# TritonDataCenter/node-zkstream

Measured on AMD Instinct MI355X. Metric: ZK ops/sec (whole node) + p50 get() RTT, 1M-znode synthetic tree, higher is better.
Workload: dtype uint8

## Files before the change

csrc/kernels/tree.hip:

```cpp
#include "zk_tree.h"
#include "zk_frame_rows.h"

namespace zk {

__global__ __launch_bounds__(TR_T) void tree_fill_k(ZkTree t, int64_t n0,
                                                   int64_t n,
                                                   const int32_t* __restrict__ nkids,
                                                   int64_t now_ms) {
  const int64_t v = n0 + (int64_t)blockIdx.x * TR_T + threadIdx.x;
  if (v >= n) return;
  const ZkNodeStore& s = t.store;
  uint8_t* slot = s.slab + s.slot_off[v];
  const int32_t dl = s.data_len[v];
  fill_stat(slot, v + 1, v + 1, now_ms, now_ms, 0, nkids[v], 0, 0, dl,
            nkids[v], v + 1);
  st_be32(slot + 68, 0);
  st_be32(slot + ZK_SLOT_LEN, dl > 0 ? dl : -1);
  t.cn[v] = cn_pack(nkids[v], nkids[v]);
  t.pzxid[v] = v + 1;
  t.eph[v] = 0;
  t.dirty[v] = 0;
}

__global__ __launch_bounds__(TR_T) void free_count_k(ZkTree t,
                                                    int64_t* __restrict__ bsum) {
  __shared__ int32_t c[TR_T / 64];
  const int64_t nn = min(t.counters[TC_NODES], t.store.cap);
  const int64_t v = (int64_t)blockIdx.x * TR_T + threadIdx.x;
  const bool f = v < nn && t.node_parent[v] == NODE_FREE;
  const uint64_t m = __ballot(f);
  if ((threadIdx.x & 63) == 0) c[threadIdx.x >> 6] = __popcll(m);
  __syncthreads();
  if (threadIdx.x == 0) {
    int64_t s = 0;
    for (int k = 0; k < TR_T / 64; ++k) s += c[k];
    bsum[blockIdx.x] = s;
  }
}

__global__ __launch_bounds__(TR_T) void free_scatter_k(
    ZkTree t, const int64_t* __restrict__ bbase,
    const int64_t* __restrict__ total) {
  __shared__ int32_t c[TR_T / 64];
  const int64_t head = t.counters[TC_FREE_HEAD];
  const int64_t nn = min(t.counters[TC_NODES], t.store.cap);
  const int64_t v = (int64_t)blockIdx.x * TR_T + threadIdx.x;
  const bool f = v < nn && t.node_parent[v] == NODE_FREE;
  const uint64_t m = __ballot(f);
  const int w = threadIdx.x >> 6;
  if ((threadIdx.x & 63) == 0) c[w] = __popcll(m);
  __syncthreads();
  int64_t r = bbase[blockIdx.x] +
              __builtin_amdgcn_mbcnt_hi((uint32_t)(m >> 32),
                                        __builtin_amdgcn_mbcnt_lo((uint32_t)m, 0));
  for (int k = 0; k < w; ++k) r += c[k];
  if (f) t.free_list[(head + r) % t.free_cap] = v;
  if (blockIdx.x == 0 && threadIdx.x == 0) {
    t.counters[TC_FREE_TAIL] = head + *total;
    t.counters[TC_FREE_PUB] = head + *total;
  }
}

__global__ __launch_bounds__(TR_T) void tree_build_k(ZkTree t, int64_t n0,
                                                    int64_t n) {
  const int64_t v = n0 + (int64_t)blockIdx.x * TR_T + threadIdx.x;
  if (v >= n || t.node_parent[v] == NODE_FREE) return;
  tree_insert(t, v, t.path_arena + t.node_path_off[v], t.node_path_len[v],
              t.store.data_len[v]);
}

}

extern "C" {

int zk_tree_fill(const ZkTree* t, int64_t n0, int64_t n, const int32_t* nkids,
                 int64_t now_ms, hipStream_t st) {
  if (n <= n0) return 0;
  const int64_t m = n - n0;
  zk::tree_fill_k<<<(unsigned)((m + zk::TR_T - 1) / zk::TR_T), zk::TR_T, 0,
                    st>>>(*t, n0, n, nkids, now_ms);
  ZK_LAUNCH_CHECK();
  return 0;
}

int64_t zk_tree_free_workspace(int64_t cap) {
  const int64_t nb = (cap + zk::TR_T - 1) / zk::TR_T;
  return 2 * nb + 8 + zk_scan_workspace(nb);
}

int zk_tree_free_compact(const ZkTree* t, int64_t* ws, hipStream_t st) {
  const int64_t nb = (t->store.cap + zk::TR_T - 1) / zk::TR_T;
  if (nb <= 0) return 0;
  int64_t* bsum = ws;
  int64_t* bbase = ws + nb;
  int64_t* total = ws + 2 * nb;
  zk::free_count_k<<<(unsigned)nb, zk::TR_T, 0, st>>>(*t, bsum);
  ZK_LAUNCH_CHECK();
  int rc = zk_scan_excl_i64(bsum, bbase, nb, total, ws + 2 * nb + 8, st);
  if (rc) return rc;
  zk::free_scatter_k<<<(unsigned)nb, zk::TR_T, 0, st>>>(*t, bbase, total);
  ZK_LAUNCH_CHECK();
  return 0;
}

int zk_tree_ht_reset(const ZkTree* t, hipStream_t st) {
  return hipMemsetAsync(t->ht, 0, (size_t)(t->mask + 1) * zk::HT_W * 8, st);
}

int zk_tree_build(const ZkTree* t, int64_t n0, int64_t n, hipStream_t st) {
  if (n <= n0) return 0;
  const int64_t m = n - n0;
  zk::tree_build_k<<<(unsigned)((m + zk::TR_T - 1) / zk::TR_T), zk::TR_T, 0,
                     st>>>(*t, n0, n);
  ZK_LAUNCH_CHECK();
  return 0;
}

}

namespace zk {

ZK_DEV void put_seq10(uint8_t* d, int32_t x) {
  uint32_t u = (uint32_t)x;
#pragma unroll
  for (int k = 9; k >= 0; --k) { d[k] = (uint8_t)('0' + u % 10); u /= 10; }
}

struct Lane {
  int32_t op, err, pl, dl, flags, dlen;
  int64_t node, zx, par, slot;
  const uint8_t* path;
};

ZK_DEV int64_t served_reply_size(int32_t op, int32_t err, int32_t dl,
                                 int32_t rpl) {
  const int64_t sz = 4 + 16;
  if (err != ERR_OK) return sz;
  switch (op) {
    case OP_GET_DATA: return sz + 4 + max(dl, 0) + STAT_BYTES;
    case OP_EXISTS: case OP_SET_DATA: return sz + STAT_BYTES;
    case OP_CREATE: return sz + 4 + max(rpl, 0);
    default: return sz;
  }
}

ZK_DEV int32_t seq_num(const ZkTree& t, int64_t i) {
  if (t.seqno == nullptr) return -1;
  const int64_t x = t.seqno[i];
  return x < 0 ? -1 : (int32_t)(uint32_t)x;
}
ZK_DEV int64_t seq_par(const ZkTree& t, int64_t i) {
  return t.seqno == nullptr || t.seqno[i] < 0 ? -1 : t.seqno[i] >> 32;
}

ZK_DEV int32_t do_create(const ZkTree& t, Lane& L, const uint8_t* data,
                         int32_t nacl, int64_t session, int64_t now_ms,
                         int64_t v, int64_t i) {
  const ZkNodeStore& s = t.store;
  const bool eph = L.flags & CF_EPHEMERAL, seq = L.flags & CF_SEQUENTIAL;
  const int32_t pre = seq ? seq_num(t, i) : -1;
  if (nacl <= 0) return ERR_INVALID_ACL;
  if (v < 0) return ERR_SYSTEM;
  const int64_t vpo = t.node_path_off[v];
  const int64_t vso = s.slot_off[v];
  const uint8_t* path = L.path;
  const int32_t pl = L.pl;
  int32_t cut = pl - 1;
  while (cut > 0 && path[cut] != '/') --cut;
  const int64_t par = cut > 0 ? tree_find(t, path, cut) : -1;
  if (cut > 0 && par < 0) return ERR_NO_NODE;
  if (par >= 0 && t.eph[par] != 0)
    return ERR_NO_CHILDREN_FOR_EPHEMERALS;
  const int32_t npl = pl + (seq ? 10 : 0);
  const bool taken = seq && par >= 0 && pre < 0;
  const int32_t seqno = !seq || par < 0 ? 0
                        : pre >= 0      ? pre
                                        : cn_cver(cn_add(t, par, 1, 1));
  uint8_t* pd = t.path_arena + vpo;
  copy_bytes(pd, path, pl);
  if (seq) put_seq10(pd + pl, seqno);
  const int32_t dl = L.dl;
  uint8_t* slot = s.slab + vso;
  fill_stat(slot, L.zx, L.zx, now_ms, now_ms, 0, 0, 0, eph ? session : 0, dl,
            0, L.zx);
  st_be32(slot + ZK_SLOT_LEN, dl > 0 ? dl : -1);
  copy_bytes(slot + ZK_SLOT_DATA, data, dl);
  t.node_path_len[v] = npl;
  s.data_len[v] = dl;
  t.cn[v] = 0;
  t.pzxid[v] = L.zx;
  t.node_parent[v] = par;
  t.node_pw[v] = pw_pack(pd - t.path_arena, npl);
  const int64_t ins = pre >= 0 ? tree_insert<true>(t, v, pd, npl, dl, vso)
                               : tree_insert(t, v, pd, npl, dl, vso);
  if (ins != v) {
    if (taken) cn_add(t, par, 0, -1);
    return ins < 0 ? ERR_SYSTEM : ERR_NODE_EXISTS;
  }
  t.eph[v] = eph ? session : 0;
  if (par >= 0) {
    if (seq) {
      atomicMax((unsigned long long*)&t.pzxid[par], (unsigned long long)L.zx);
    } else {
      parent_touch(t, par, 1, true, L.zx);
    }
  }
  L.par = par;
  L.node = v;
  L.slot = s.slot_off[v];
  return ERR_OK;
}

struct ServeSegs : ZkSegs {};
static_assert(TR_T == FR_T, "a workgroup per block of FR_T frames");
template <bool PARSE, bool RO, bool TILES, bool MS = false, bool DEFER = false>
ZK_DEV void tree_serve_body(
    const ZkTree& t, const uint8_t* __restrict__ rx, const ZkReqOut& q,
    const int64_t* __restrict__ foff, const int32_t* __restrict__ flen,
    const int64_t* __restrict__ n_dev, int64_t ncap, int32_t* __restrict__ r_op,
    int32_t* __restrict__ r_xid, int32_t* __restrict__ r_err,
    int64_t* __restrict__ r_node, int64_t* __restrict__ r_zxid,
    int64_t* __restrict__ r_path_off, int32_t* __restrict__ r_path_len,
    int64_t* __restrict__ r_slot, int64_t* __restrict__ r_sizes,
    int64_t* __restrict__ r_bsum, int64_t session, int64_t now_ms,
    const uint8_t* __restrict__ rank, int32_t pass, int32_t last_pass,
    int64_t snap_base, int64_t snap_cap, int64_t* __restrict__ snap_top,
    int32_t wslot, int64_t* __restrict__ fired, const ZkFrameTiles* T,
    int64_t* __restrict__ rows_off, int32_t* __restrict__ rows_len,
    const ServeSegs* M = nullptr) {
  session = sess_of(t, session);
  const uint32_t blk = xcd_remap(blockIdx.x, gridDim.x);
  const int64_t i = (int64_t)blk * TR_T + threadIdx.x;
  const bool in_batch = i < ncap && i < *n_dev;
  int64_t fo = 0;
  int32_t fl = 0;
  if (TILES) {
    __shared__ FrLds rows;
    const int64_t nf = *n_dev;
    if (fr_row(*T, blk, nf < ncap ? nf : ncap, rows, fo, fl)) {
      rows_off[i] = fo;
      rows_len[i] = fl;
    }
    fr_housekeep(*T);
  }
  const int32_t rb = rank != nullptr && in_batch ? (int32_t)rank[i] : 0;
  const int32_t rk = rb & ORD_RANK;
  const bool live = in_batch && (rk == pass || (last_pass && rk > pass));
  int32_t ms_err = ERR_OK;
  if (MS && live) {
    const int64_t sg = M->f_seg[i];
    if (*M->bad != 0 || sg < 0 || sg >= M->S) {
      ms_err = ERR_SYSTEM;
    } else {
      session = sess_of(t, M->sessions[sg]);
      wslot = M->wslots[sg];
      if (M->seg_state[sg] == 1) ms_err = ERR_SESSION_EXPIRED;
    }
  }
  const bool refused = live && (rk > pass || (MS && ms_err != ERR_OK));
  ReqFields rq{ST_BAD_DECODE, 0, OP_PING, 0, 0, 0, 0, -1, -1, -1, 0};
  if (live) {
    if (PARSE) {
      rq = TILES ? parse_request(rx, fo, fl)
                 : parse_request(rx, foff[i], flen[i]);
    } else {
      rq.status = q.status[i];
      rq.xid = q.xid[i];
      rq.op = q.opcode[i];
      rq.arg = q.arg[i];
      rq.pl = q.path_len[i];
      rq.dl = q.data_len[i];
      rq.vc = q.vec_count[i];
      rq.poff = q.path_off[i];
      rq.doff = q.data_off[i];
    }
  }
  const bool ok_req = live && !refused && rq.status == ST_OK;
  const ZkNodeStore& s = t.store;
  Lane L;
  L.op = live ? rq.op : OP_PING;
  L.err = refused ? (MS && ms_err != ERR_OK ? ms_err : ERR_SYSTEM)
                  : (live && !ok_req ? ERR_BAD_ARGUMENTS : ERR_OK);
  L.node = -1;
  L.slot = -1;
  L.dlen = 0;
  L.par = -1;
  L.flags = 0;
  L.path = nullptr;
  L.pl = L.dl = 0;
  if (ok_req) {
    L.path = rx + rq.poff;
    L.pl = rq.pl;
    L.dl = max(rq.dl, 0);
    L.flags = rq.arg;
  }
  const bool write = ok_req && (L.op == OP_CREATE || L.op == OP_SET_DATA ||
                                L.op == OP_DELETE);
  const int64_t zbase = t.counters[TC_ZXID];
  L.zx = write ? zbase + i + 1 : zbase;
  const bool create = !RO && ok_req && L.op == OP_CREATE;
  int64_t v = -1;
  int32_t npl = 0, cap = 0;
  if (create) {
    npl = L.pl + ((L.flags & CF_SEQUENTIAL) ? 10 : 0);
    cap = max(L.dl, 128);
  }
  if (RO && ok_req && L.op != OP_GET_DATA && L.op != OP_EXISTS)
    L.err = ERR_UNIMPLEMENTED;
  if (!RO) {
    const int64_t pub = t.counters[TC_FREE_PUB];
    const int64_t h = block_ticket(&t.counters[TC_FREE_HEAD], create);
    if (create && h < pub) v = t.free_list[h % t.free_cap];
    const bool fresh = create && v < 0;
    const int64_t nv = block_ticket(&t.counters[TC_NODES], fresh);
    if (fresh && nv < s.cap) v = nv;
    const bool new_path = v >= 0 && (fresh || npl > t.node_path_cap[v]);
    const bool new_slot = v >= 0 && (fresh || cap > s.slot_cap[v]);
    const int32_t pcap = (npl + 15) & ~15;
    const int64_t po = wave_bytes(&t.counters[TC_PATH_TOP],
                                  new_path ? pcap : 0);
    const int64_t sb = new_slot ? slot_bytes(cap) : 0;
    const int64_t so = wave_bytes(&t.counters[TC_SLAB_TOP], sb);
    if (new_path) {
      if (po + pcap <= t.path_cap) {
        t.node_path_off[v] = po;
        t.node_path_len[v] = npl;
        t.node_path_cap[v] = pcap;
      } else {
        t.node_path_len[v] = 0;
        t.node_path_cap[v] = 0;
      }
    }
    if (new_slot) {
      if (so + sb <= t.slab_cap) {
        s.slot_off[v] = so;
        s.slot_cap[v] = cap;
      } else {
        s.slot_cap[v] = -1;
      }
    }
    if (v >= 0 && ((new_path && po + pcap > t.path_cap) ||
                   (new_slot && so + sb > t.slab_cap))) {
      L.err = ERR_SYSTEM;
    }
  }
  int64_t freed = -1;
  bool numbered = !RO && live && seq_num(t, i) >= 0;
  if (ok_req && L.err == ERR_OK) {
    switch (L.op) {
      case OP_GET_DATA: case OP_EXISTS:
        {
          const Found f = tree_lookup<true>(t, L.path, L.pl);
          L.node = f.node;
          L.slot = f.slot;
          L.dlen = f.dlen;
        }
        if (L.node < 0) L.err = ERR_NO_NODE;
        break;
      case OP_SET_DATA: {
        const Found f = tree_lookup(t, L.path, L.pl);
        const int64_t node = f.node;
        if (node < 0) { L.err = ERR_NO_NODE; break; }
        L.slot = f.slot;
        if (L.dl > s.slot_cap[node]) { L.err = ERR_BAD_ARGUMENTS; break; }
        uint8_t* slot = s.slab + L.slot;
        unsigned int* ver = (unsigned int*)(slot + 32);
        const int32_t want = L.flags;
        unsigned int old = *ver, cmp;
        do {
          cmp = old;
          if (want != -1 && cmp != bswap32((uint32_t)want)) break;
          old = atomicCAS(ver, cmp, bswap32(bswap32(cmp) + 1));
        } while (old != cmp);
        if (old != cmp || (want != -1 && cmp != bswap32((uint32_t)want))) {
          L.err = ERR_BAD_VERSION;
          break;
        }
        copy_bytes(slot + ZK_SLOT_DATA, rx + rq.doff, L.dl);
        st_be32(slot + ZK_SLOT_LEN, L.dl > 0 ? L.dl : -1);
        s.data_len[node] = L.dl;
        ent_set_dlen(t, f.ent, L.dl);
        st_be64(slot + 8, L.zx);
        st_be64(slot + 24, now_ms);
        st_be32(slot + 52, L.dl);
        L.node = node;
        break;
      }
      case OP_CREATE:
        L.err = do_create(t, L, rx + rq.doff, rq.vc, session,
                          now_ms, v, i);
        if (L.err == ERR_OK) numbered = false;
        if (L.err == ERR_OK && r_path_off != nullptr) {
          r_path_off[i] = t.node_path_off[v];
          r_path_len[i] = t.node_path_len[v];
        }
        break;
      case OP_DELETE: {
        const Found f = tree_lookup(t, L.path, L.pl);
        const int64_t node = f.node, so = f.slot;
        if (node < 0) { L.err = ERR_NO_NODE; break; }
        const int32_t nkids = cn_nchild(__hip_atomic_load(
            &t.cn[node], __ATOMIC_RELAXED, __HIP_MEMORY_SCOPE_AGENT));
        const int32_t want = L.flags;
        if (want != -1 && ld_be32(s.slab + so + 32) != want) {
          L.err = ERR_BAD_VERSION;
          break;
        }
        if (nkids > 0) {
          L.err = ERR_NOT_EMPTY;
          break;
        }
        if (!tree_erase_at(t, f.ent, node)) { L.err = ERR_NO_NODE; break; }
        L.par = t.node_parent[node];
        if (L.par >= 0) parent_touch(t, L.par, -1, true, L.zx);
        t.eph[node] = 0;
        freed = node;
        break;
      }
      case OP_SYNC: case OP_PING:
        break;
      case OP_SET_WATCHES:
        break;
      default:
        L.err = ERR_UNIMPLEMENTED;
    }
  }
  if (numbered)
    cn_add(t, seq_par(t, i),
           MS && ms_err == ERR_SYSTEM && !(DEFER && rk == ORD_RANK) ? -1 : 0,
           -1);
  if (t.wt_key != nullptr && ok_req) {
    const bool wflag = rq.arg == 1;
    if (L.op == OP_GET_DATA && wflag && L.err == ERR_OK) {
      wt_arm(t, L.path, L.pl, WK_DATA, wslot);
    } else if (L.op == OP_EXISTS && wflag &&
               (L.err == ERR_OK || L.err == ERR_NO_NODE)) {
      wt_arm(t, L.path, L.pl, WK_DATA, wslot);
    } else if (L.err == ERR_OK && (L.op == OP_SET_DATA ||
                                   L.op == OP_CREATE ||
                                   L.op == OP_DELETE)) {
      const int64_t node = L.op == OP_DELETE ? freed : L.node;
      const int64_t pw = t.node_pw[node];
      const int64_t ppw = L.par >= 0 ? t.node_pw[L.par] : 0;
      const uint8_t* np = node_path(t, pw);
      const int32_t nl = pw_len(pw);
      uint64_t m0 = wt_fire(t, np, nl, WK_DATA), m1 = 0, m2 = 0;
      if (L.op == OP_DELETE) m1 = wt_fire(t, np, nl, WK_CHILD) & ~m0;
      if (L.op != OP_SET_DATA && L.par >= 0)
        m2 = wt_fire(t, node_path(t, ppw), pw_len(ppw), WK_CHILD);
      if (fired != nullptr) {
        int64_t* f = fired + (int64_t)WT_REC * i;
        f[0] = (int64_t)m0;
        f[1] = (int64_t)m1;
        f[2] = (int64_t)m2;
        f[3] = pw;
        f[4] = ppw;
      }
    }
  }
  if (rank != nullptr) {
    const bool snap = (rb & ORD_SNAP) && live && L.err == ERR_OK &&
                      (L.op == OP_GET_DATA || L.op == OP_EXISTS ||
                       L.op == OP_SET_DATA);
    const int64_t dl = snap && L.op == OP_GET_DATA ? L.dlen : 0;
    const int64_t sb = snap ? slot_bytes((int32_t)dl) : 0;
    const int64_t so = wave_bytes(snap_top, sb);
    if (snap) {
      if (so + sb <= snap_cap) {
        copy_bytes(s.slab + snap_base + so, s.slab + L.slot,
                   (int32_t)(ZK_SLOT_DATA + dl));
        L.slot = snap_base + so;
      } else {
        L.err = ERR_SYSTEM;
      }
    }
  }
  if (create && L.err != ERR_OK && v >= 0) freed = v;
  if (!RO) {
    wave_free(t, freed);
    wave_mark_dirty(t, L.err == ERR_OK ? L.par
                       : DEFER && numbered ? seq_par(t, i) : -1);
  }
  if (r_sizes != nullptr) {
    __shared__ int64_t sm[TR_T / 64 + 1];
    int64_t sz = 0;
    if (live) {
      const bool get = L.err == ERR_OK && L.op == OP_GET_DATA;
      const bool mk = L.err == ERR_OK && L.op == OP_CREATE;
      sz = served_reply_size(L.op, L.err, get ? L.dlen : 0,
                             mk ? t.node_path_len[L.node] : 0);
      r_sizes[i] = sz;
    } else if (in_batch && rk < pass) {
      sz = r_sizes[i];
    } else if (!in_batch && i < ncap) {
      r_sizes[i] = 0;
    }
    int64_t tot;
    block_excl_scan(sz, sm, &tot);
    if (threadIdx.x == 0) r_bsum[blk] = tot;
  }
  if (!live) return;
  r_op[i] = L.op;
  r_xid[i] = rq.xid;
  r_err[i] = L.err;
  r_node[i] = L.op == OP_DELETE ? -1 : L.node;
  r_zxid[i] = L.zx;
  if (r_slot != nullptr) r_slot[i] = L.op == OP_DELETE ? -1 : L.slot;
}

template <bool PARSE, bool RO = false>
__global__ __launch_bounds__(TR_T) void tree_serve_k(
    ZkTree t, const uint8_t* __restrict__ rx, ZkReqOut q,
    const int64_t* __restrict__ foff, const int32_t* __restrict__ flen,
    const int64_t* __restrict__ n_dev, int64_t ncap, int32_t* __restrict__ r_op,
    int32_t* __restrict__ r_xid, int32_t* __restrict__ r_err,
    int64_t* __restrict__ r_node, int64_t* __restrict__ r_zxid,
    int64_t* __restrict__ r_path_off, int32_t* __restrict__ r_path_len,
    int64_t* __restrict__ r_slot, int64_t* __restrict__ r_sizes,
    int64_t* __restrict__ r_bsum, int64_t session, int64_t now_ms,
    const uint8_t* __restrict__ rank, int32_t pass, int32_t last_pass,
    int64_t snap_base, int64_t snap_cap, int64_t* __restrict__ snap_top,
    int32_t wslot, int64_t* __restrict__ fired) {
  tree_serve_body<PARSE, RO, false>(
      t, rx, q, foff, flen, n_dev, ncap, r_op, r_xid, r_err, r_node, r_zxid,
      r_path_off, r_path_len, r_slot, r_sizes, r_bsum, session, now_ms, rank,
      pass, last_pass, snap_base, snap_cap, snap_top, wslot, fired, nullptr,
      nullptr, nullptr);
}

template <bool RO>
__global__ __launch_bounds__(TR_T) void tree_serve_tiles_k(
    ZkTree t, ZkFrameTiles T, int64_t* __restrict__ rows_off,
    int32_t* __restrict__ rows_len, const int64_t* __restrict__ n_dev,
    int64_t ncap, ZkServeOut o, int64_t session, int64_t now_ms,
    int32_t wslot, int64_t* __restrict__ fired) {
  tree_serve_body<true, RO, true>(
      t, T.buf, ZkReqOut{}, nullptr, nullptr, n_dev, ncap, o.opcode, o.xid,
      o.err, o.node, o.zxid, o.path_off, o.path_len, o.slot, o.sizes,
      o.block_sums, session, now_ms, nullptr, 0, 1, 0, 0, nullptr, wslot,
      fired, &T, rows_off, rows_len);
}

template <bool PARSE>
__global__ __launch_bounds__(TR_T) void tree_serve_sess_k(
    ZkTree t, const uint8_t* __restrict__ rx, ZkReqOut q,
    const int64_t* __restrict__ foff, const int32_t* __restrict__ flen,
    const int64_t* __restrict__ n_dev, int64_t ncap, ZkServeOut o,
    int64_t now_ms, const uint8_t* __restrict__ rank, int32_t pass,
    int32_t last_pass, int64_t snap_base, int64_t snap_cap,
    int64_t* __restrict__ snap_top, int64_t* __restrict__ fired,
    ServeSegs M) {
  tree_serve_body<PARSE, false, false, true>(
      t, rx, q, foff, flen, n_dev, ncap, o.opcode, o.xid, o.err, o.node,
      o.zxid, o.path_off, o.path_len, o.slot, o.sizes, o.block_sums, 0,
      now_ms, rank, pass, last_pass, snap_base, snap_cap, snap_top, -1, fired,
      nullptr, nullptr, nullptr, &M);
}

__global__ __launch_bounds__(TR_T) void tree_serve_sess_defer_k(
    ZkTree t, const uint8_t* __restrict__ rx, ZkReqOut q,
    const int64_t* __restrict__ n_dev, int64_t ncap, ZkServeOut o,
    int64_t now_ms, const uint8_t* __restrict__ rank, int32_t pass,
    int32_t last_pass, int64_t snap_base, int64_t snap_cap,
    int64_t* __restrict__ snap_top, int64_t* __restrict__ fired,
    ServeSegs M) {
  tree_serve_body<false, false, false, true, true>(
      t, rx, q, nullptr, nullptr, n_dev, ncap, o.opcode, o.xid, o.err, o.node,
      o.zxid, o.path_off, o.path_len, o.slot, o.sizes, o.block_sums, 0,
      now_ms, rank, pass, last_pass, snap_base, snap_cap, snap_top, -1, fired,
      nullptr, nullptr, nullptr, &M);
}

int serve_launch(const ServeLaunch& s, hipStream_t st) {
  if (s.ncap <= 0) return 0;
  const ZkServeOut& o = *s.out;
  if ((o.sizes == nullptr) != (o.block_sums == nullptr)) return -1;
  if (s.tiles != nullptr) {
    if (s.q != nullptr || s.rank != nullptr || s.segs != nullptr) return -1;
    const auto kt = s.read_only ? tree_serve_tiles_k<true>
                                : tree_serve_tiles_k<false>;
    kt<<<(unsigned)((s.ncap + TR_T - 1) / TR_T), TR_T, 0, st>>>(
        *s.tree, *s.tiles, s.rows_off, s.rows_len, s.n_dev, s.ncap, o,
        s.session, s.now_ms, s.wslot, s.fired);
    ZK_LAUNCH_CHECK();
    return 0;
  }
  const bool parse = s.q == nullptr;
  if (s.segs != nullptr) {
    const ServeSegs M{*s.segs};
    if (s.read_only || M.f_seg == nullptr || M.sessions == nullptr ||
        M.wslots == nullptr || M.seg_state == nullptr || M.bad == nullptr ||
        M.S < 1)
      return -1;
    if (s.defer) {
      if (parse || s.rank == nullptr) return -1;
      tree_serve_sess_defer_k<<<(unsigned)((s.ncap + TR_T - 1) / TR_T), TR_T,
                                0, st>>>(
          *s.tree, s.rx, *s.q, s.n_dev, s.ncap, o, s.now_ms, s.rank, s.pass,
          s.last_pass, s.snap_base, s.snap_cap, s.snap_top, s.fired, M);
      ZK_LAUNCH_CHECK();
      return 0;
    }
    const auto km = parse ? tree_serve_sess_k<true> : tree_serve_sess_k<false>;
    km<<<(unsigned)((s.ncap + TR_T - 1) / TR_T), TR_T, 0, st>>>(
        *s.tree, s.rx, parse ? ZkReqOut{} : *s.q, s.foff, s.flen, s.n_dev,
        s.ncap, o, s.now_ms, s.rank, s.pass, s.last_pass, s.snap_base,
        s.snap_cap, s.snap_top, s.fired, M);
    ZK_LAUNCH_CHECK();
    return 0;
  }
  const auto k = !parse        ? tree_serve_k<false>
                 : s.read_only ? tree_serve_k<true, true>
                               : tree_serve_k<true>;
  k<<<(unsigned)((s.ncap + TR_T - 1) / TR_T), TR_T, 0, st>>>(
      *s.tree, s.rx, parse ? ZkReqOut{} : *s.q, s.foff, s.flen, s.n_dev,
      s.ncap, o.opcode, o.xid, o.err, o.node, o.zxid, o.path_off, o.path_len,
      o.slot, o.sizes, o.block_sums, s.session, s.now_ms, s.rank, s.pass,
      s.last_pass, s.snap_base, s.snap_cap, s.snap_top, s.wslot, s.fired);
  ZK_LAUNCH_CHECK();
  return 0;
}

}

extern "C" {

int zk_tree_serve(const ZkTree* t, const uint8_t* rx, const ZkReqOut* q,
                  const int64_t* n_dev, int64_t ncap, const ZkServeOut* out,
                  int64_t session, int64_t now_ms, hipStream_t st) {
  if (ncap <= 0) return 0;
  zk::ServeLaunch s;
  s.tree = t, s.rx = rx, s.q = q, s.n_dev = n_dev, s.ncap = ncap;
  s.out = out, s.session = session, s.now_ms = now_ms;
  const int rc = zk::serve_launch(s, st);
  return rc ? rc : zk::finish_launch(t, n_dev, 0, 1, st);
}

int zk_tree_serve_frames(const ZkTree* t, const uint8_t* rx,
                         const int64_t* foff, const int32_t* flen,
                         const int64_t* n_dev, int64_t ncap,
                         const ZkServeOut* out, int64_t session,
                         int64_t now_ms, int32_t wslot, int64_t* fired,
                         int32_t read_only, hipStream_t st) {
  zk::ServeLaunch s;
  s.tree = t, s.rx = rx, s.foff = foff, s.flen = flen, s.n_dev = n_dev;
  s.ncap = ncap, s.out = out, s.session = session, s.now_ms = now_ms;
  s.wslot = wslot, s.fired = fired, s.read_only = read_only;
  return zk::serve_launch(s, st);
}

int zk_tree_serve_frames_sessions(
    const ZkTree* t, const uint8_t* rx, const int64_t* foff,
    const int32_t* flen, const int64_t* n_dev, int64_t ncap,
    const ZkServeOut* out, int64_t now_ms, int64_t* fired, const ZkSegs* segs,
    hipStream_t st) {
  if (segs == nullptr) return (int)hipErrorInvalidValue;
  zk::ServeLaunch s;
  s.tree = t, s.rx = rx, s.foff = foff, s.flen = flen, s.n_dev = n_dev;
  s.ncap = ncap, s.out = out, s.now_ms = now_ms, s.fired = fired;
  s.segs = segs;
  return zk::serve_launch(s, st);
}

int zk_tree_serve_tiles(const ZkTree* t, const ZkFrameTiles* tiles,
                        int64_t* foff, int32_t* flen, const int64_t* n_dev,
                        int64_t ncap, const ZkServeOut* out, int64_t session,
                        int64_t now_ms, int32_t wslot, int64_t* fired,
                        int32_t read_only, hipStream_t st) {
  if (ncap <= 0) return (int)hipErrorInvalidValue;
  zk::ServeLaunch s;
  s.tree = t, s.rx = tiles->buf, s.tiles = tiles, s.rows_off = foff;
  s.rows_len = flen, s.n_dev = n_dev, s.ncap = ncap, s.out = out;
  s.session = session, s.now_ms = now_ms, s.wslot = wslot, s.fired = fired;
  s.read_only = read_only;
  return zk::serve_launch(s, st);
}

}

namespace zk {

constexpr int FIN_T = 1024;

ZK_DEV void finish_body(const ZkTree& t, const int64_t* n_dev,
                        int64_t bump_zxid, int32_t publish) {
  int64_t* c = t.counters;
  const int64_t nd = __hip_atomic_load(&c[TC_DIRTY], __ATOMIC_RELAXED,
                                       __HIP_MEMORY_SCOPE_AGENT);
  for (int64_t k = threadIdx.x; k < nd; k += blockDim.x) {
    const int64_t p = __hip_atomic_load(&t.dirty_list[k], __ATOMIC_RELAXED,
                                        __HIP_MEMORY_SCOPE_AGENT);
    uint8_t* slot = t.store.slab + t.store.slot_off[p];
    const int64_t cn = __hip_atomic_load(&t.cn[p], __ATOMIC_RELAXED,
                                         __HIP_MEMORY_SCOPE_AGENT);
    st_be32(slot + 36, cn_cver(cn));
    st_be32(slot + 56, cn_nchild(cn));
    st_be64(slot + 60, __hip_atomic_load(&t.pzxid[p], __ATOMIC_RELAXED,
                                         __HIP_MEMORY_SCOPE_AGENT));
    t.dirty[p] = 0;
  }
  __syncthreads();
  if (threadIdx.x != 0) return;
  auto ld = [&](int k) {
    return __hip_atomic_load(&c[k], __ATOMIC_RELAXED, __HIP_MEMORY_SCOPE_AGENT);
  };
  if (publish) {
    if (ld(TC_FREE_HEAD) > ld(TC_FREE_PUB)) c[TC_FREE_HEAD] = ld(TC_FREE_PUB);
    c[TC_FREE_PUB] = ld(TC_FREE_TAIL);
  }
  c[TC_DIRTY] = 0;
  c[TC_ZXID] = ld(TC_ZXID) + (n_dev != nullptr ? *n_dev : bump_zxid);
}

template <int NT = FIN_T>
__global__ __launch_bounds__(NT) void tree_finish_k(ZkTree t,
                                                   const int64_t* n_dev,
                                                   int64_t bump_zxid,
                                                   int32_t publish) {
  finish_body(t, n_dev, bump_zxid, publish);
}

template <int NT>
__global__ __launch_bounds__(NT) void tree_finish_scan_k(
    ZkTree t, const int64_t* n_dev, int64_t bump_zxid, int32_t publish,
    const int64_t* __restrict__ bsum, int64_t nb, int64_t* __restrict__ bbase,
    int64_t* __restrict__ total) {
  if (blockIdx.x == 0) {
    finish_body(t, n_dev, bump_zxid, publish);
    return;
  }
  constexpr int FS_V = 8;
  __shared__ int64_t sm[NT / 64 + 1];
  int64_t carry = 0;
  for (int64_t c0 = 0; c0 < nb; c0 += (int64_t)NT * FS_V) {
    const int64_t b = c0 + (int64_t)threadIdx.x * FS_V;
    int64_t v[FS_V];
    int64_t s = 0;
#pragma unroll
    for (int j = 0; j < FS_V; ++j) {
      v[j] = b + j < nb ? bsum[b + j] : 0;
      s += v[j];
    }
    int64_t tot;
    int64_t p = carry + block_excl_scan(s, sm, &tot);
#pragma unroll
    for (int j = 0; j < FS_V; ++j) {
      if (b + j < nb) bbase[b + j] = p;
      p += v[j];
    }
    carry += tot;
  }
  if (threadIdx.x == 0) *total = carry;
}

template <bool DBG, bool WT>
ZK_DEV void tree_expire_body(
    const ZkTree& t, int64_t session, int64_t ncap,
    unsigned long long* __restrict__ removed, int32_t* __restrict__ dbg,
    int64_t* __restrict__ rec, int64_t rec_cap) {
  session = sess_of(t, session);
  const int64_t v = (int64_t)blockIdx.x * TR_T + threadIdx.x;
  const int64_t c0 = DBG ? (int64_t)wall_clock64() : 0;
  int64_t c1 = 0, c2 = 0;
  bool hit = v < ncap && v < t.counters[TC_NODES] && t.eph[v] == session;
  const int64_t zx = t.counters[TC_ZXID] + 1;
  int64_t par = -1;
  int32_t dflag = 1;
  if (hit) {
    const int64_t poff = t.node_path_off[v];
    const int32_t plen = t.node_path_len[v];
    const int64_t p0 = t.node_parent[v];
    if (p0 >= 0)
      dflag = __hip_atomic_load(&t.dirty[p0], __ATOMIC_RELAXED,
                                __HIP_MEMORY_SCOPE_AGENT);
    const int64_t tag = tomb_tag(zx);
    const int64_t es = tree_erase_slot(t, v, t.path_arena + poff, plen, tag);
    hit = es >= 0;
    if (DBG) c1 = (int64_t)wall_clock64();
    if (hit) {
      ht_shift(t, es, session, tag);
      if (DBG) c2 = (int64_t)wall_clock64();
      par = p0;
      if (par >= 0) parent_touch(t, par, -1, true, zx);
      t.eph[v] = 0;
      if (WT) {
        const int64_t ws = wt_find(t, t.path_arena + poff, plen);
        const uint64_t m0 = wt_fire_at(t, ws, WK_DATA);
        const uint64_t m1 = wt_fire_at(t, ws, WK_CHILD) & ~m0;
        const int64_t ppw = par >= 0 ? t.node_pw[par] : 0;
        const uint64_t m2 =
            par >= 0 ? wt_fire(t, node_path(t, ppw), pw_len(ppw), WK_CHILD)
                     : 0;
        if ((m0 | m1 | m2) != 0 && rec != nullptr) {
          const int64_t k = (int64_t)atomicAdd((unsigned long long*)&rec[0],
                                               1ull);
          if (k < rec_cap) {
            int64_t* f = rec + 8 + (int64_t)WT_REC * k;
            f[0] = (int64_t)m0;
            f[1] = (int64_t)m1;
            f[2] = (int64_t)m2;
            f[3] = pw_pack(poff, plen);
            f[4] = ppw;
          }
        }
      }
    }
  }
  wave_free(t, hit ? v : -1, removed);
  wave_mark_dirty_at(t, par, dflag);
  if (DBG && hit) {
    const int64_t c3 = (int64_t)wall_clock64();
    dbg[4 * v] = (int32_t)c0;
    dbg[4 * v + 1] = (int32_t)(c1 - c0);
    dbg[4 * v + 2] = (int32_t)(c2 - c1);
    dbg[4 * v + 3] = (int32_t)(c3 - c0);
  }
}

template <bool DBG>
__global__ __launch_bounds__(TR_T) void tree_expire_k(
    ZkTree t, int64_t session, int64_t ncap,
    unsigned long long* __restrict__ removed, int32_t* __restrict__ dbg) {
  tree_expire_body<DBG, false>(t, session, ncap, removed, dbg, nullptr, 0);
}

__global__ __launch_bounds__(TR_T) void tree_expire_wt_k(
    ZkTree t, int64_t session, int64_t ncap,
    unsigned long long* __restrict__ removed, int64_t* __restrict__ rec,
    int64_t rec_cap) {
  tree_expire_body<false, true>(t, session, ncap, removed, nullptr, rec,
                                rec_cap);
}

int finish_launch(const ZkTree* t, const int64_t* n_dev, int64_t bump,
                  int32_t publish, hipStream_t st) {
  tree_finish_k<256><<<1, 256, 0, st>>>(*t, n_dev, bump, publish);
  ZK_LAUNCH_CHECK();
  return 0;
}

}

extern "C" {

int zk_tree_finish_scan(const ZkTree* t, const int64_t* n_dev, int64_t bump,
                        int32_t publish, int64_t ncap, int64_t* scan_ws,
                        int64_t* total, hipStream_t st) {
  const int64_t nb = ncap > 0 ? (ncap + 255) / 256 : 0;
  zk::tree_finish_scan_k<256><<<2, 256, 0, st>>>(
      *t, n_dev, bump, publish, scan_ws, nb, scan_ws + nb, total);
  ZK_LAUNCH_CHECK();
  return 0;
}

static int32_t* g_exp_dbg = nullptr;
void zk_tree_expire_debug(int32_t* buf) { g_exp_dbg = buf; }

int zk_tree_expire(const ZkTree* t, int64_t session, int64_t ncap,
                   unsigned long long* removed, int64_t* rec, int64_t rec_cap,
                   hipStream_t st) {
  if (ncap <= 0) return 0;
  const unsigned nb = (unsigned)((ncap + zk::TR_T - 1) / zk::TR_T);
  if (t->wt_key != nullptr)
    zk::tree_expire_wt_k<<<nb, zk::TR_T, 0, st>>>(*t, session, ncap, removed,
                                                  rec, rec_cap);
  else if (g_exp_dbg != nullptr)
    zk::tree_expire_k<true><<<nb, zk::TR_T, 0, st>>>(*t, session, ncap, removed,
                                                     g_exp_dbg);
  else
    zk::tree_expire_k<false><<<nb, zk::TR_T, 0, st>>>(*t, session, ncap,
                                                      removed, nullptr);
  ZK_LAUNCH_CHECK();
  return zk::finish_launch(t, nullptr, 1, 1, st);
}

}

namespace zk {

ZK_DEV uint64_t wave_sum_u64(uint64_t x) {
#pragma unroll
  for (int d = 32; d >= 1; d >>= 1) x += __shfl_xor(x, d, 64);
  return x;
}

__global__ __launch_bounds__(TR_T) void tree_digest_k(
    ZkTree t, unsigned long long* __restrict__ out) {
  const int64_t v = (int64_t)blockIdx.x * TR_T + threadIdx.x;
  const int64_t nn = min(t.counters[TC_NODES], t.store.cap);
  uint64_t h = 0, live = 0;
  if (v < nn && t.node_parent[v] != NODE_FREE) {
    const int64_t pw = t.node_pw[v];
    const uint8_t* slot = t.store.slab + t.store.slot_off[v];
    const int32_t dl = t.store.data_len[v];
    h = path_hash(node_path(t, pw), pw_len(pw));
    auto mix = [&](uint64_t x) {
      h = (h ^ x) * 0x9E3779B97F4A7C15ull;
      h ^= h >> 29;
    };
    mix((uint64_t)ld_be64(slot));
    mix((uint64_t)ld_be64(slot + 8));
    mix((uint32_t)ld_be32(slot + 32));
    mix((uint64_t)t.cn[v]);
    mix((uint64_t)t.pzxid[v]);
    mix((uint64_t)t.eph[v]);
    mix((uint64_t)(uint32_t)dl);
    mix(path_hash(slot + ZK_SLOT_DATA, max(dl, 0)));
    live = 1;
  }
  h = wave_sum_u64(h);
  live = wave_sum_u64(live);
  if ((threadIdx.x & 63) == 0 && live) {
    atomicAdd(&out[0], (unsigned long long)h);
    atomicAdd(&out[1], (unsigned long long)live);
  }
}

__global__ __launch_bounds__(TR_T) void ht_census_k(
    ZkTree t, unsigned long long* __restrict__ out) {
  uint64_t used = 0, tomb = 0;
  for (int64_t s = (int64_t)blockIdx.x * TR_T + threadIdx.x; s <= t.mask;
       s += (int64_t)gridDim.x * TR_T) {
    if (*ht_key(t, s) != 0) {
      ++used;
      if (val_tomb(*ht_val(t, s))) ++tomb;
    }
  }
  used = wave_sum_u64(used);
  tomb = wave_sum_u64(tomb);
  if ((threadIdx.x & 63) == 0) {
    atomicAdd(&out[2], (unsigned long long)used);
    atomicAdd(&out[3], (unsigned long long)tomb);
  }
}

int digest_launch(const ZkTree* t, unsigned long long* out, hipStream_t st) {
  const int64_t nb = (t->store.cap + TR_T - 1) / TR_T;
  if (nb <= 0) return 0;
  tree_digest_k<<<(unsigned)nb, TR_T, 0, st>>>(*t, out);
  ZK_LAUNCH_CHECK();
  return 0;
}

}

extern "C" {

int zk_tree_digest(const ZkTree* t, unsigned long long* out, hipStream_t st) {
  if (hipMemsetAsync(out, 0, 32, st) != hipSuccess) return -4;
  const int64_t nb = (t->store.cap + zk::TR_T - 1) / zk::TR_T;
  if (nb > 0) {
    zk::tree_digest_k<<<(unsigned)nb, zk::TR_T, 0, st>>>(*t, out);
    ZK_LAUNCH_CHECK();
  }
  zk::ht_census_k<<<2048, zk::TR_T, 0, st>>>(*t, out);
  ZK_LAUNCH_CHECK();
  return 0;
}

}
```

csrc/kernels/zk_frame_rows.h:

```cpp
#pragma once
#include "zk_common.h"

namespace zk {

constexpr int FT_S = 4096;
constexpr int FT_LMAX = FT_S / 4;
constexpr int FT_STAGE = FT_S + 16;
constexpr int FK_T = 64;
constexpr int FL_NB = 2;
constexpr int FL_GW = FL_NB + 1;
constexpr int LW_MINS = 4, LW_LAST = 6, LW_NOSPEC = 7, LW_GRID = 8;
constexpr int LW_BIG = 16;
constexpr int LW_END = 32;
static_assert(LW_GRID + FL_GW <= LW_BIG, "grid words");
constexpr int FR_T = 256;
constexpr int FR_W = 64;

ZK_DEV int64_t stream_len(const int64_t* n_dev, int64_t n_cap) {
  if (n_dev == nullptr) return n_cap;
  const int64_t v = *n_dev;
  return v < 0 ? 0 : (v < n_cap ? v : n_cap);
}

ZK_DEV int32_t lds_be32(const uint8_t* sb, int32_t p) {
  const int32_t a = p & ~3;
  const uint32_t lo = *(const uint32_t*)(sb + a);
  const uint32_t hi = *(const uint32_t*)(sb + a + 4);
  return (int32_t)bswap32(__builtin_amdgcn_alignbyte(hi, lo, p & 3));
}

ZK_DEV int32_t m_cnt(int64_t m) { return (int32_t)(m & 0x7FF); }
ZK_DEV int32_t m_np(int64_t m) { return (int32_t)((m >> 11) & 0x7FF); }
ZK_DEV int32_t m_js(int64_t m) { return (int32_t)((m >> 22) & 0x7FF) - 1; }
ZK_DEV bool m_term(int64_t m) { return (m >> 33) & 1; }
ZK_DEV bool m_bad(int64_t m) { return (m >> 34) & 1; }
constexpr int64_t M_STALE = (int64_t)1 << 35;
ZK_DEV bool m_stale(int64_t m) { return (m >> 35) & 1; }

template <int WIN>
ZK_DEV void fc_stage(const uint8_t* __restrict__ buf, int64_t n, int64_t wb,
                     uint8_t* win, int lane) {
  constexpr int PER = WIN / 1024;
  uint4 v[PER];
#pragma unroll
  for (int j = 0; j < PER; ++j) {
    const int64_t g = wb + 16 * (lane + 64 * j);
    v[j] = make_uint4(0, 0, 0, 0);
    if (g + 16 <= n) {
      __builtin_memcpy(&v[j], buf + g, 16);
    } else if (g < n) {
      uint8_t* b = (uint8_t*)&v[j];
      for (int k = 0; k < 16; ++k) b[k] = g + k < n ? buf[g + k] : 0;
    }
  }
#pragma unroll
  for (int j = 0; j < PER; ++j) *(uint4*)(win + 16 * (lane + 64 * j)) = v[j];
  __builtin_amdgcn_wave_barrier();
  asm volatile("s_waitcnt lgkmcnt(0)" ::: "memory");
  __builtin_amdgcn_wave_barrier();
}

ZK_DEV void fr_stage_lean(const uint8_t* __restrict__ buf, int64_t n,
                          int64_t wb, uint8_t* win, int lane) {
#pragma unroll 1
  for (int j = 0; j < FT_S / 1024; ++j) {
    const int64_t g = wb + 16 * (lane + 64 * j);
    uint4 v = make_uint4(0, 0, 0, 0);
    if (g + 16 <= n) {
      __builtin_memcpy(&v, buf + g, 16);
    } else if (g < n) {
      uint32_t w[4] = {0, 0, 0, 0};
#pragma unroll 1
      for (int k = 0; k < 16; ++k)
        if (g + k < n) w[k >> 2] |= (uint32_t)buf[g + k] << (8 * (k & 3));
      v = make_uint4(w[0], w[1], w[2], w[3]);
    }
    *(uint4*)(win + 16 * (lane + 64 * j)) = v;
  }
  __builtin_amdgcn_wave_barrier();
  asm volatile("s_waitcnt lgkmcnt(0)" ::: "memory");
  __builtin_amdgcn_wave_barrier();
}

ZK_DEV void fr_bounds(const uint16_t* __restrict__ list,
                      const uint16_t* __restrict__ pre, int64_t t, int64_t m,
                      int64_t x, int32_t k, int64_t& p, int64_t& q) {
  const int32_t cnt = m_cnt(m), np = m_np(m), js = m_js(m);
  const int64_t ts = t * FT_S;
  const uint16_t* P = pre + t * FT_LMAX;
  const uint16_t* R = list + t * FT_LMAX + (js < 0 ? 0 : js);
  p = ts + (k < np ? P[k] : R[k - np]);
  const int32_t k1 = k + 1;
  q = k1 < cnt ? ts + (k1 < np ? P[k1] : R[k1 - np]) : x;
}

template <bool LEAN, typename Emit>
ZK_DEV void fr_walk_stale(const uint8_t* __restrict__ buf, int64_t n,
                          int64_t t, int32_t c, int32_t cnt, int64_t x,
                          uint8_t* sb, int lane, Emit emit) {
  const int64_t ts = t * FT_S;
  if (LEAN) fr_stage_lean(buf, n, ts, sb, lane);
  else fc_stage<FT_S>(buf, n, ts, sb, lane);
  if (lane == 0) {
    uint8_t* pb = sb + FT_S;
#pragma unroll 1
    for (int k = 0; k < 16; ++k)
      pb[k] = ts + FT_S + k < n ? buf[ts + FT_S + k] : 0;
  }
  __builtin_amdgcn_wave_barrier();
  asm volatile("s_waitcnt lgkmcnt(0)" ::: "memory");
  int32_t ent = 0;
  for (int32_t k = 0; k < cnt; ++k) {
    ent = lane == (k & 63) ? c : ent;
    const int32_t len = __builtin_amdgcn_readfirstlane(lds_be32(sb, c));
    c += 4 + len;
    if ((k & 63) == 63 || k == cnt - 1) {
      const int32_t last = k & 63;
      const int32_t nxt = __shfl_down(ent, 1, 64);
      if (lane <= last) {
        const int64_t p = ts + ent;
        const int64_t q = lane < last ? ts + nxt
                                      : (k == cnt - 1 ? x : ts + c);
        emit((k & ~63) + lane, p, q);
      }
    }
  }
}


struct FrLds {
  __attribute__((aligned(16))) uint8_t stage[FT_STAGE];
  int64_t off[FR_T];
  int32_t len[FR_T];
  int32_t rb[FR_W];
  unsigned long long pick;
};

ZK_DEV int64_t fr_rowbase(const ZkFrameTiles& T, int64_t t) {
  return T.bsum[t / FK_T] + T.base[t];
}

ZK_DEV bool fr_row(const ZkFrameTiles& T, uint32_t blk, int64_t nrows,
                   FrLds& S, int64_t& foff, int32_t& flen) {
  const int tid = threadIdx.x, lane = tid & 63;
  const int64_t i0 = (int64_t)blk * FR_T;
  if (i0 >= nrows) return false;
  const bool act = i0 + tid < nrows;
  const int64_t n = stream_len(T.n_dev, T.n_cap);
  const int64_t lastk = *T.lastk;
  int64_t w0;
  {
    const int64_t b = T.fblk[blk];
    const int64_t t = b * FK_T + lane;
    const bool le = t <= lastk && fr_rowbase(T, t) <= i0;
    const uint64_t m = __ballot(le);
    w0 = b * FK_T + (m ? 63 - (int64_t)__builtin_clzll(m) : 0);
  }
  int64_t t = -1;
  int32_t k = 0;
  bool placed = !act;
  for (;;) {
    if (tid < FR_W) {
      const int64_t tw = w0 + tid;
      int32_t r = 0x7FFFFFFF;
      if (tw <= lastk) {
        const int64_t d = fr_rowbase(T, tw) - i0;
        r = d > FR_T ? FR_T : (int32_t)d;
      }
      S.rb[tid] = r;
    }
    __syncthreads();
    if (!placed) {
      int lo = 0;
#pragma unroll
      for (int s = FR_W / 2; s >= 1; s >>= 1)
        if (S.rb[lo + s] <= tid) lo += s;
      if (lo < FR_W - 1 || w0 + FR_W - 1 >= lastk) {
        t = w0 + lo;
        k = tid - S.rb[lo];
        placed = true;
      }
    }
    if (!__syncthreads_or(!placed)) break;
    w0 += FR_W - 1;
  }
  int64_t m = 0, x = 0;
  bool stale = false;
  if (act) {
    m = T.rec_meta[t];
    x = T.rec_exit[t];
    stale = m_stale(m);
    foff = 0;
    flen = 0;
    if (!stale && (uint32_t)k < (uint32_t)m_cnt(m)) {
      int64_t p, q;
      fr_bounds(T.list, T.pre, t, m, x, k, p, q);
      foff = p + 4;
      flen = (int32_t)(q - p - 4);
    }
  }
  if (__syncthreads_or(stale)) {
    for (;;) {
      if (tid == 0) S.pick = ~0ull;
      __syncthreads();
      if (stale) atomicMin(&S.pick, (unsigned long long)t);
      __syncthreads();
      const unsigned long long pk = S.pick;
      if (pk == ~0ull) break;
      const int64_t tt = (int64_t)pk;
      if (stale && t == tt) {
        S.off[tid] = 0;
        S.len[tid] = 0;
      }
      __syncthreads();
      if (tid < 64) {
        const int64_t mt = T.rec_meta[tt];
        const int64_t rel = fr_rowbase(T, tt) - i0;
        const int32_t c = __builtin_amdgcn_readfirstlane(
            (int32_t)(T.rec_entry[tt] - tt * FT_S));
        fr_walk_stale<true>(T.buf, n, tt, c, m_cnt(mt), T.rec_exit[tt], S.stage,
                      lane, [&](int32_t kk, int64_t p, int64_t q) {
                        const int64_t r = rel + kk;
                        if (r >= 0 && r < FR_T) {
                          S.off[r] = p + 4;
                          S.len[r] = (int32_t)(q - p - 4);
                        }
                      });
      }
      __syncthreads();
      if (stale && t == tt) {
        foff = S.off[tid];
        flen = S.len[tid];
        stale = false;
      }
      __syncthreads();
    }
  }
  return act;
}

ZK_DEV void fr_housekeep(const ZkFrameTiles& T) {
  const int64_t n = stream_len(T.n_dev, T.n_cap);
  const int64_t ntiles = (n + FT_S - 1) / FT_S;
  const int64_t step = (int64_t)gridDim.x * blockDim.x;
  for (int64_t t = (int64_t)blockIdx.x * blockDim.x + threadIdx.x; t < ntiles;
       t += step) {
    T.lbw[2 * t] = 0;
    T.lbw[2 * t + 1] = 0;
  }
  if (blockIdx.x == 0) {
    uint64_t* tail = T.lbw + 2 * T.tiles;
    const int tid = threadIdx.x;
    if (tid == 0) {
      tail[LW_MINS] = 0;
      tail[LW_MINS + 1] = 0;
      tail[LW_NOSPEC] = 0;
      tail[LW_GRID + FL_NB] = 0;
    }
    if (tid < LW_END - LW_BIG) tail[LW_BIG + tid] = 0;
  }
}

}
```

Measured before the change: 2.105 billion.

## Stage each wave's request frame span into LDS before parsing in read-only serve

In the read-only tiled serve path, each wave computes the contiguous byte span covering its lanes' frames. If the span fits in a 4 KiB budget, the wave copies it into shared memory with aligned 16-byte loads and points parsing and path access at that copy. This replaces scattered byte-wise global reads during request parsing and path hashing with one coalesced load followed by LDS reads. The cost is 16 KiB of extra LDS per workgroup, which may lower occupancy, plus extra registers for the staged vectors. L.path now points into LDS, so any later use of it after the copy's lifetime or across waves could be a risk.

Result: faster. 2.173 billion, median of 6 (+3.2%).

```diff
diff --git a/csrc/kernels/tree.hip b/csrc/kernels/tree.hip
--- a/csrc/kernels/tree.hip
+++ b/csrc/kernels/tree.hip
@@ -213,6 +213,7 @@
 
 struct ServeSegs : ZkSegs {};
 static_assert(TR_T == FR_T, "a workgroup per block of FR_T frames");
+constexpr int SRV_STAGE = 4096;
 template <bool PARSE, bool RO, bool TILES, bool MS = false, bool DEFER = false>
 ZK_DEV void tree_serve_body(
     const ZkTree& t, const uint8_t* __restrict__ rx, const ZkReqOut& q,
@@ -234,14 +235,28 @@
   const bool in_batch = i < ncap && i < *n_dev;
   int64_t fo = 0;
   int32_t fl = 0;
+  const uint8_t* rxs = rx;
   if (TILES) {
     __shared__ FrLds rows;
     const int64_t nf = *n_dev;
-    if (fr_row(*T, blk, nf < ncap ? nf : ncap, rows, fo, fl)) {
+    const bool has = fr_row(*T, blk, nf < ncap ? nf : ncap, rows, fo, fl);
+    if (has) {
       rows_off[i] = fo;
       rows_len[i] = fl;
     }
     fr_housekeep(*T);
+    if constexpr (RO && TILES) {
+      __shared__ __attribute__((aligned(16)))
+          uint8_t img[TR_T / 64][fr_image_bytes<SRV_STAGE>()];
+      uint8_t* im = img[threadIdx.x >> 6];
+      const int lane = threadIdx.x & 63;
+      const int64_t n = stream_len(T->n_dev, T->n_cap);
+      FrSpan<SRV_STAGE> F;
+      fr_span_load(rx, n, has, fo, fl, lane, F);
+      int32_t rel;
+      if (fr_span_store(rx, n, F, im, lane, fo, rel))
+        rxs = (const uint8_t*)((uintptr_t)(const uint8_t*)im + rel - fo);
+    }
   }
   const int32_t rb = rank != nullptr && in_batch ? (int32_t)rank[i] : 0;
   const int32_t rk = rb & ORD_RANK;
@@ -261,7 +276,7 @@
   ReqFields rq{ST_BAD_DECODE, 0, OP_PING, 0, 0, 0, 0, -1, -1, -1, 0};
   if (live) {
     if (PARSE) {
-      rq = TILES ? parse_request(rx, fo, fl)
+      rq = TILES ? parse_request(rxs, fo, fl)
                  : parse_request(rx, foff[i], flen[i]);
     } else {
       rq.status = q.status[i];
@@ -289,7 +304,7 @@
   L.path = nullptr;
   L.pl = L.dl = 0;
   if (ok_req) {
-    L.path = rx + rq.poff;
+    L.path = rxs + rq.poff;
     L.pl = rq.pl;
     L.dl = max(rq.dl, 0);
     L.flags = rq.arg;
diff --git a/csrc/kernels/zk_frame_rows.h b/csrc/kernels/zk_frame_rows.h
--- a/csrc/kernels/zk_frame_rows.h
+++ b/csrc/kernels/zk_frame_rows.h
@@ -1,5 +1,6 @@
 #pragma once
 #include "zk_common.h"
+#include "zk_stage_span.h"
 
 namespace zk {
 
@@ -80,6 +81,90 @@
   __builtin_amdgcn_wave_barrier();
   asm volatile("s_waitcnt lgkmcnt(0)" ::: "memory");
   __builtin_amdgcn_wave_barrier();
+}
+
+template <int N>
+ZK_DEV void lds_words(const uint8_t* sb, int32_t p, uint32_t (&w)[N]) {
+  const uint32_t* a = (const uint32_t*)(sb + (p & ~3));
+  uint32_t r[N + 1];
+#pragma unroll
+  for (int k = 0; k <= N; ++k) r[k] = a[k];
+#pragma unroll
+  for (int k = 0; k < N; ++k)
+    w[k] = __builtin_amdgcn_alignbyte(r[k + 1], r[k], p & 3);
+}
+
+ZK_DEV int64_t wave_uniform(int64_t x) {
+  const uint32_t lo = __builtin_amdgcn_readfirstlane((uint32_t)x);
+  const uint32_t hi =
+      __builtin_amdgcn_readfirstlane((uint32_t)((uint64_t)x >> 32));
+  return (int64_t)(((uint64_t)hi << 32) | lo);
+}
+
+template <int IMG>
+constexpr int fr_image_bytes() { return IMG + 16; }
+
+template <int IMG>
+struct FrSpan {
+  static_assert(IMG % 1024 == 0, "whole chunks a lane");
+  static constexpr int PER = IMG / 1024;
+  StageSpan sp;
+  int64_t s;
+  bool ok;
+  uint4 v[PER];
+};
+
+template <int IMG>
+ZK_DEV void fr_span_load(const uint8_t* __restrict__ buf, int64_t n, bool mine,
+                         int64_t fo, int32_t fl, int lane, FrSpan<IMG>& F) {
+  F.ok = false;
+  const uint64_t m = __ballot(mine);
+  if (m == 0) return;
+  const int first = (int)__builtin_ctzll(m);
+  const int last = 63 - (int)__builtin_clzll(m);
+  const int64_t s = wave_uniform(__shfl(fo, first, 64));
+  const int64_t e = wave_uniform(__shfl(fo + (fl > 0 ? fl : 0), last, 64));
+  if (!span_fits(s, e, n, IMG)) return;
+  const bool in = !mine || (fl >= 0 && fo >= s && fo + fl <= e);
+  if (__ballot(!in) != 0) return;
+  F.sp = span_make((uint64_t)(uintptr_t)buf, s, e, n);
+  F.s = s;
+  if (!span_image_fits(F.sp, IMG)) return;
+  F.ok = true;
+  if (F.sp.clipped) return;
+#pragma unroll
+  for (int j = 0; j < FrSpan<IMG>::PER; ++j) {
+    const int32_t c = lane + 64 * j;
+    F.v[j] = make_uint4(0, 0, 0, 0);
+    if (c < F.sp.nchunks)
+      __builtin_memcpy(&F.v[j], buf + span_chunk_off(F.sp, c), 16);
+  }
+}
+
+template <int IMG>
+ZK_DEV bool fr_span_store(const uint8_t* __restrict__ buf, int64_t n,
+                          const FrSpan<IMG>& F, uint8_t* img, int lane,
+                          int64_t fo, int32_t& rel) {
+  if (!F.ok) return false;
+  if (!F.sp.clipped) {
+#pragma unroll
+    for (int j = 0; j < FrSpan<IMG>::PER; ++j) {
+      const int32_t c = lane + 64 * j;
+      if (c < F.sp.nchunks) *(uint4*)(img + 16 * c) = F.v[j];
+    }
+  } else {
+#pragma unroll 1
+    for (int32_t c = lane; c < F.sp.nchunks; c += 64) {
+      uint32_t w[4];
+      span_load_chunk(buf, n, F.sp, c, w);
+      *(uint4*)(img + 16 * c) = make_uint4(w[0], w[1], w[2], w[3]);
+    }
+  }
+  __builtin_amdgcn_wave_barrier();
+  asm volatile("s_waitcnt lgkmcnt(0)" ::: "memory");
+  __builtin_amdgcn_wave_barrier();
+  rel = F.sp.head + (int32_t)(fo - F.s);
+  return true;
 }
 
 ZK_DEV void fr_bounds(const uint16_t* __restrict__ list,
diff --git a/csrc/kernels/zk_stage_span.h b/csrc/kernels/zk_stage_span.h
--- /dev/null
+++ b/csrc/kernels/zk_stage_span.h
@@ -0,0 +1,49 @@
+#pragma once
+#include <stdint.h>
+
+#include "zk_wire.h"
+
+namespace zk {
+
+struct StageSpan {
+  int64_t off0;
+  int32_t head;
+  int32_t nchunks;
+  bool clipped;
+};
+
+ZK_HD bool span_fits(int64_t s, int64_t e, int64_t n, int64_t budget) {
+  return s >= 0 && s <= e && e <= n && e - s <= budget;
+}
+
+ZK_HD StageSpan span_make(uint64_t base, int64_t s, int64_t e, int64_t n) {
+  StageSpan sp;
+  sp.head = (int32_t)((base + (uint64_t)s) & 15);
+  sp.off0 = s - sp.head;
+  sp.nchunks = (int32_t)((sp.head + (e - s) + 15) >> 4);
+  sp.clipped = sp.off0 < 0 || sp.off0 + 16 * (int64_t)sp.nchunks > n;
+  return sp;
+}
+
+ZK_HD bool span_image_fits(const StageSpan& sp, int64_t img_bytes) {
+  return 16 * (int64_t)sp.nchunks <= img_bytes;
+}
+
+ZK_HD int64_t span_chunk_off(const StageSpan& sp, int32_t c) {
+  return sp.off0 + 16 * (int64_t)c;
+}
+
+ZK_HD void span_load_chunk(const uint8_t* buf, int64_t n, const StageSpan& sp,
+                           int32_t c, uint32_t (&w)[4]) {
+  const int64_t g = span_chunk_off(sp, c);
+  if (g >= 0 && g + 16 <= n) {
+    __builtin_memcpy(w, buf + g, 16);
+    return;
+  }
+  w[0] = w[1] = w[2] = w[3] = 0;
+  for (int k = 0; k < 16; ++k)
+    if (g + k >= 0 && g + k < n)
+      w[k >> 2] |= (uint32_t)buf[g + k] << (8 * (k & 3));
+}
+
+}
```
